# lgleznah/mort

Measured on AMD Instinct MI355X. Metric: Msamples/sec (width x height x spp/s), Scene 1 1200x675, higher is better.
Workload: dtype f32; 1 GPU; Scene 1 (random-spheres cover) 1200x675, 500 spp nominal = 484 effective, depth 20, megakernel, seed 69420, host LCG scene; mode=mega, partition=rows/8 interleaved over 1 rank(s)

## Files before the change

mort_amd/csrc/hip/debug.hip:

```cpp
#include <hip/hip_runtime.h>

#include <array>
#include <cstring>
#include <thread>
#include <vector>

#include "mort_hip.h"
#include "mega_bvh.h"
#include "scene_blob.h"
#include "mort_ctx.h"
#include "world_images.h"
#include "dev_radiance.h"
#include "query_common.h"

#pragma clang fp contract(off)

extern "C" int mort_hip_debug_wave_log(mort_ctx *c, unsigned long long *out, size_t max_waves) {
    if (!c || !out || !c->d_wave_log) return 0;
    hipSetDevice(c->device);
    quiesce(c);
    const size_t n = c->wave_log_waves < max_waves ? c->wave_log_waves : max_waves;
    if (hipMemcpy(out, c->d_wave_log, n * 16 * sizeof(unsigned long long), hipMemcpyDeviceToHost) != hipSuccess) return 0;
    return (int)n;
}
// ... 255 lines not shown
    if (hipSetDevice(device) != hipSuccess) return MORT_ERR_NO_DEVICE;
    float *d_in = nullptr;
    unsigned long long *d_out = nullptr;
    int st = MORT_OK;
    if (hipMalloc((void **)&d_in, n * per * sizeof(float)) != hipSuccess || hipMalloc((void **)&d_out, 16 * sizeof(unsigned long long)) != hipSuccess) st = MORT_ERR_NOMEM;
    if (st == MORT_OK && (hipMemcpy(d_in, in, n * per * sizeof(float), hipMemcpyHostToDevice) != hipSuccess ||
                          hipMemset(d_out, 0, 16 * sizeof(unsigned long long)) != hipSuccess)) st = MORT_ERR_HIP;
    if (st == MORT_OK) {
        const size_t blocks = (n + 255) / 256;
        exact_forms_kernel<<<dim3((unsigned)(blocks < 4096 ? blocks : 4096)), dim3(256)>>>(what, d_in, n, d_out);
        if (hipGetLastError() != hipSuccess || hipDeviceSynchronize() != hipSuccess ||
            hipMemcpy(out, d_out, 16 * sizeof(unsigned long long), hipMemcpyDeviceToHost) != hipSuccess) st = MORT_ERR_HIP;
    }
    if (d_in) (void)hipFree(d_in);
    if (d_out) (void)hipFree(d_out);
    if (caller_device >= 0 && caller_device != device) (void)hipSetDevice(caller_device);
    return st;
}

extern "C" int mort_hip_debug_bvh_lds_levels(const mort_world *w, int *out) {
    if (!w || !out) return MORT_ERR_INVALID;
    SceneBlob sb;
    const int st = build_scene_blob(w, sb);
    if (st != MORT_OK) return st;
    const mortc::Compiled &o = sb.comp;
    for (int i = 0; i < 4; i++) out[i] = 0;
    if (!one_sphere_bvh(o) || o.own_nodes.empty() || o.own_nodes4.empty()) return MORT_OK;
    BvhImages im;
    build_bvh_images(o, im);
    if (!im.fits) return MORT_OK;
    const uint32_t levels = (uint32_t)(o.own4_stack > 1 ? o.own4_stack : 1) + MORT_BVH_TSTACK_SPARE;
    const int shapes[3] = {1024, 768, 256};
    out[0] = (int)im.fb.size();
    for (int k = 0; k < 3; k++) { uint32_t a = 0, b = 0; out[1 + k] = state_lds_levels((uint32_t)im.fb.size(), shapes[k], levels, 1024u, a, b); }
    return MORT_OK;
}


__device__ __forceinline__ int mort_f2i_select(float x) {
    const bool in_range = (x > -2147483648.0f) && (x < 2147483648.0f);
    const int t = (int)(in_range ? x : 0.0f);
    return (x != x) ? 0 : (x >= 2147483648.0f) ? 2147483647 : (x <= -2147483648.0f) ? (-2147483647 - 1) : t;
}
static __global__ void __launch_bounds__(256) f2i_all_kernel(unsigned long long *out) {
    const uint32_t first = blockIdx.x * 256u + threadIdx.x;
    uint32_t differ = 0, lowest = 0xffffffffu;
    for (uint32_t k = 0; k < 4096u; k++) {
        const uint32_t bits = first + (k << 20);
        const float x = __uint_as_float(bits);
        if (mort_f2i(x) != mort_f2i_select(x)) { differ++; lowest = bits < lowest ? bits : lowest; }
    }
    atomicAdd(&out[2], 4096ull);
    if (differ) { atomicAdd(&out[0], (unsigned long long)differ); atomicMin(&out[1], (unsigned long long)lowest); }
}
static __global__ void __launch_bounds__(256) f2i_list_kernel(const uint32_t *bits, size_t n, int *res) {
    const size_t i = (size_t)blockIdx.x * 256 + threadIdx.x;
    if (i < n) res[i] = mort_f2i(__uint_as_float(bits[i]));
}

extern "C" int mort_hip_debug_f2i_device(int device, const uint32_t *bits, size_t n, int *res, unsigned long long *out) {
    if (!out || (n && (!bits || !res)) || n > ((size_t)1 << 28)) return MORT_ERR_INVALID;
    int caller_device = -1;
    if (hipGetDevice(&caller_device) != hipSuccess) caller_device = -1;
    if (hipSetDevice(device) != hipSuccess) return MORT_ERR_NO_DEVICE;
    uint32_t *d_bits = nullptr;
    int *d_res = nullptr;
    unsigned long long *d_out = nullptr;
// ... 514 lines not shown
```

mort_amd/csrc/hip/mega_bvh.h:

```cpp
#ifndef MORT_MEGA_BVH_H
#define MORT_MEGA_BVH_H

#include "dev_render.h"


struct FastArgs {
    RenderArgs r;
    const unsigned char *hot_src;
    uint32_t hot_bytes;
    uint32_t off_nodes4, off_leafrecs, off_lambert, off_metal, off_diel, off_dlight, off_iso, off_solid, off_checker;
    uint32_t off_tstack;
    int node_first, node_count;
    unsigned int *next_q;
    int tiles_x, tiles_total;
    uint32_t off_stack;
    int stack_lds_depth;
    const unsigned *tile_order;
    int gen_tiles;
    int spread_shift;
    unsigned *tile_cost;
    int th_s, th_l, t_keep;
    int sub;
    float *vaccum;
    float4 *deep;
// ... 370 lines not shown
#define TS_AT(ptr) (*(ptr))
    const DLambert *lambert = (const DLambert *)(lds + BU_U(L.off_lambert));
    const DMetal *metal = (const DMetal *)(lds + BU_U(L.off_metal));
    const DDielectric *dielectric = (const DDielectric *)(lds + BU_U(L.off_diel));
    const DLambert *dlight = (const DLambert *)(lds + BU_U(L.off_dlight));
    const DLambert *isotropic = (const DLambert *)(lds + BU_U(L.off_iso));
    const DSolid *solid = (const DSolid *)(lds + BU_U(L.off_solid));
    const DChecker *checker = (const DChecker *)(lds + BU_U(L.off_checker));

    const int node_first = BU_I(L.node_first), node_end = node_first + BU_I(L.node_count);
    const int th_s = BU_I(L.th_s), th_l = BU_I(L.th_l), t_keep = BU_I(L.t_keep);
    const int sqrt_spp = BU_I(L.r.sqrt_spp), bounce_limit = BU_I(L.r.bounce_limit);
    const float bg_x = BU_F(L.r.background.x), bg_y = BU_F(L.r.background.y), bg_z = BU_F(L.r.background.z);
    const int spp = sqrt_spp * sqrt_spp;
    const unsigned total_q = (unsigned)BU_I(L.tiles_total) * 64u;

    int state = ((int)(threadIdx.x & 63u) < BU_I(L.lane_cap)) ? ST_S : ST_DONE, kind = K_NEWPIX;
    int xy = 0, lofs = 0;
    Rng rng; rng.d = rng.v0 = rng.v1 = rng.v2 = rng.v3 = rng.v4 = 0; rng.draws = 0;
    V3 pixel_color = mk(0, 0, 0);
    int s_ij = 0, iter = 0;
    uint32_t segments = 0;
    Ray ray; ray.o = mk(0, 0, 0); ray.d = mk(0, 0, 1); ray.tm = 0;
    float ray_time0 = 0;
    OwnRay orr; orr.ix = orr.iy = orr.iz = 1; orr.mx = orr.my = orr.mz = 0; orr.band = 0; orr.invlen = 1;
    float ray_a = 1, closest = 0;
    float ray_a_rcp = 1;
    int best = -1;
    uint32_t node = 0;
    unsigned short *spa = ts_base;
    int flags = 0;
    DeepPtr stack_deep = (DeepPtr)BU_P(L.deep) + ((size_t)blockIdx.x * BLOCK + threadIdx.x);
    const size_t deep_stride = (size_t)gridDim.x * BLOCK;
    unsigned long long ident_mask = 0ull;
    float4 *stack_lds = (float4 *)(lds + BU_U(L.off_stack));
    const int DL = BU_I(L.stack_lds_depth);
#ifdef MORT_PROFILE_STATES
    unsigned long long *const counters_p = fap->r.counters;
    unsigned long long prof[6] = {0, 0, 0, 0, 0, 0};
    unsigned long long prof_truns = 0;
    unsigned long long profc[8] = {0, 0, 0, 0, 0, 0, 0, 0};
    unsigned long long ps0 = 0, ps1;
#define PROFS0() do { ps0 = __builtin_readcyclecounter(); } while (0)
#define PROFS(i) do { ps1 = __builtin_readcyclecounter(); profc[i] += ps1 - ps0; ps0 = ps1; } while (0)
    unsigned long long pt0 = __builtin_readcyclecounter(), pt1;
    const unsigned long long prof_r0 = __builtin_amdgcn_s_memrealtime();
#define PROF(i, lanes) do { prof[2 * (i)] += 1; prof[2 * (i) + 1] += (unsigned long long)(lanes); } while (0)
    unsigned long long profb[12] = {0, 0, 0, 0, 0, 0, 0, 0, 0, 0, 0, 0};
#ifdef MORT_PROFILE_FINE
#define PROFB(i) do { } while (0)
    unsigned long long proff[12] = {0, 0, 0, 0, 0, 0, 0, 0, 0, 0, 0, 0};
#define PROFF(i) do { ps1 = __builtin_readcyclecounter(); proff[i] += ps1 - ps0; profc[4] += ps1 - ps0; ps0 = ps1; } while (0)
#else
#define PROFF(i) do { } while (0)
#define PROFB(i) do { const unsigned long long m_ = __ballot(1); if ((int)(threadIdx.x & 63) == __ffsll((long long)m_) - 1) { \
        atomicAdd(&counters_p[18 + 2 * (i)], 1ull); atomicAdd(&counters_p[19 + 2 * (i)], (unsigned long long)__popcll(m_)); } } while (0)
#endif
#define PROFC(i) do { pt1 = __builtin_readcyclecounter(); profc[i] += pt1 - pt0; pt0 = pt1; } while (0)
#else
#define PROF(i, lanes) do { } while (0)
#define PROFB(i) do { } while (0)
#define PROFF(i) do { } while (0)
#define PROFC(i) do { } while (0)
#define PROFS0() do { } while (0)
#define PROFS(i) do { } while (0)
#endif

    int leader = -1;
    const bool drain_rounds = DRAIN && BU_I(L.drain_rounds) == 1;
    const bool live_thresholds = BU_I(L.drain_rounds) == 3;
    bool running = true;
    while (running) {
      int nS = 0;
      for (;;) {
        const unsigned long long mT = __ballot(state == ST_T);
        const unsigned long long mL = __ballot(state == ST_L);
        const unsigned long long mS = __ballot(state == ST_S);
        if ((mT | mL | mS) == 0ull) { running = false; break; }
        const int nT = __popcll(mT), nL = __popcll(mL);
        nS = __popcll(mS);
        int pick;
// ... 130 lines not shown
                        atomicAdd(&fap->r.counters[3], 1ull);
                        const RefHit h = reference_walk(fap->r.sc.nodes, node_first, node_end, fap->r.sc.spheres, ray.o.x, ray.o.y, ray.o.z,
                                                        ray.d.x, ray.d.y, ray.d.z, ray.tm, ray_a);
                        best = h.best; closest = h.closest;
                    }
                    PROFF(0);
                REGION("S:hitrecord");
                    if (best < 0) {
                        final_value = mk(bg_x, bg_y, bg_z);
                        kind = K_FINISH;
                    } else {
                        DSphere sp;
                        if (need_ref) sp = fap->r.sc.spheres[best];
                        else {
                            const float4 *lp = leafrecs + (best >> 16) + ((best & 0x8000) ? 2 : 0);
                            const float4 s0 = lp[0], s1 = lp[1];
                            sp.cx = s0.x; sp.cy = s0.y; sp.cz = s0.z; sp.radius = s0.w; sp.vx = s1.x; sp.vy = s1.y; sp.vz = s1.z; sp.mat = __float_as_uint(s1.w);
                        }
                        const V3 p = ray_at(ray, closest);
                        const V3 outward = vdiv(vsub(p, sphere_center(sp, ray.tm)), sp.radius);
                        const bool front_face = vdot(ray.d, outward) < 0;
                        const V3 normal = front_face ? outward : vneg(outward);
                        const int mtype = DREF_TYPE(sp.mat), midx = DREF_IDX(sp.mat);
                        PROFF(1);
                        StackEntry e;
                        if (mtype == MORT_MAT_METAL) {
                REGION("S:metal");
                            PROFB(0);
                            const DMetal m = metal[midx];
                            V3 reflected = reflect(ray.d, normal);
                            reflected = vadd(vunit(reflected), vscale(m.fuzz, random_unit_vector(rng)));
                            ray.o = p; ray.d = reflected;
                            e.kx = 1.0f * m.r; e.ky = 1.0f * m.g; e.kz = 1.0f * m.b; e.rp = 1.0f;
                            PROFF(2);
                        } else if (mtype == MORT_MAT_DIELECTRIC) {
                REGION("S:dielectric");
                            PROFB(1);
                            const DDielectric m = dielectric[midx];
                            const float refraction_ratio = front_face ? m.inv_ior : m.ior;
                            const V3 unit_direction = vunit(ray.d);
                            const float cos_theta = (float)mort_fmin((double)vdot(vneg(unit_direction), normal), 1.0);
                            const float sin_theta = (float)mort_sqrt(1.0 - (double)(cos_theta * cos_theta));
                            const bool cant_refract = (double)(refraction_ratio * sin_theta) > 1.0;
                            V3 direction;
                            if (cant_refract || reflectance(cos_theta, refraction_ratio) > random_float(rng))
                                direction = reflect(unit_direction, normal);
                            else
                                direction = refract(unit_direction, normal, refraction_ratio);
                            ray.o = p; ray.d = direction;
                            e.kx = 1.0f; e.ky = 1.0f; e.kz = 1.0f; e.rp = 1.0f;
                            ident_mask |= (1ull << iter);
                            PROFF(3);
                        } else if (mtype == MORT_MAT_LAMBERTIAN || mtype == MORT_MAT_ISOTROPIC) {
                REGION("S:lambertian");
                            PROFB(2);
                            const bool lamb = (mtype == MORT_MAT_LAMBERTIAN);
                            const DLambert m = lamb ? lambert[midx] : isotropic[midx];
                            V3 attenuation = mk(m.r, m.g, m.b);
                            if (m.tex != 0) {
                                uint32_t tex = m.tex;
                                bool resolved = false;
                                for (int guard = 0; guard < 8 && !resolved; guard++) {
                                    const int tt = DREF_TYPE(tex), ti = DREF_IDX(tex);
                                    if (tt == MORT_TEXTURE_SOLID) { const DSolid sc = solid[ti]; attenuation = mk(sc.r, sc.g, sc.b); resolved = true; }
                                    else if (tt == MORT_TEXTURE_CHECKER) {
                                        const DChecker c = checker[ti];
                                        const int xi = mort_f2i(mort_floorf(c.inv_scale * p.x));
                                        const int yi = mort_f2i(mort_floorf(c.inv_scale * p.y));
                                        const int zi = mort_f2i(mort_floorf(c.inv_scale * p.z));
                                        tex = ((xi + yi + zi) % 2 == 0) ? c.even : c.odd;
                                    } else break;
                                }
                                if (!resolved) {
                                    const V3Ret c = texture_value_uv(&fap->r.sc, tex, outward.x, outward.y, outward.z, p.x, p.y, p.z);
                                    attenuation = mk(c.x, c.y, c.z);
                                }
                            }
                            PROFF(4);
                REGION("S:lamb_scatter");
                            V3 dir;
                            float mat_pdf, scattering_pdf;
                            if (lamb) {
                                const Onb uvw = onb_from_w(normal);
                                dir = onb_local(uvw, random_cosine_direction(rng));
                                const V3 ud = vunit(dir);
                                const float cosine_theta = vdot(ud, uvw.w);
                                mat_pdf = mort_fmaxf(0, (float)((double)cosine_theta / 3.1415926));
                                const float cos_theta = vdot(normal, ud);
                                scattering_pdf = (cos_theta < 0) ? 0.0f : (float)((double)cos_theta / 3.141592565);
                            } else {
                                dir = random_unit_vector(rng);
                                mat_pdf = (float)(1 / (4 * 3.1415926));
                                scattering_pdf = (float)(1 / (4 * 3.1415926));
                            }
                            ray.o = p; ray.d = dir; ray.tm = ray_time0;
                            e.kx = scattering_pdf * attenuation.x; e.ky = scattering_pdf * attenuation.y; e.kz = scattering_pdf * attenuation.z;
                            e.rp = 1 / mat_pdf;
                            PROFF(5);
                        } else {
                REGION("S:light");
                            V3 emission = mk(0, 0, 0);
                            if (mtype == MORT_MAT_DIFFUSE_LIGHT && front_face) {
                                const DLambert m = dlight[midx];
                                if (m.tex == 0) emission = mk(m.r, m.g, m.b);
                                else { const V3Ret c = texture_value_uv(&fap->r.sc, m.tex, outward.x, outward.y, outward.z, p.x, p.y, p.z); emission = mk(c.x, c.y, c.z); }
                            }
                            final_value = emission;
                            kind = K_FINISH;
                            PROFF(6);
                        }
                REGION("S:stackstore");
                        if (kind == K_SHADE) {
                            if (!((ident_mask >> iter) & 1ull)) {
                                float4 e4; e4.x = e.kx; e4.y = e.ky; e4.z = e.kz; e4.w = e.rp;
                                if (iter < DL) stack_lds[iter * BLOCK + threadIdx.x] = e4;
                                else stack_deep[(size_t)(iter - DL) * deep_stride] = DeepEntry{e4.x, e4.y, e4.z, e4.w};
                            }
                            iter++;
                            if (iter >= bounce_limit) { final_value = mk(0, 0, 0); kind = K_FINISH; }
                        }
                    }
                }
                REGION("S:finish");
                PROFS(4);
                if (kind == K_FINISH) {
                    PROFB(3);
                    if (iter > 0) {
                        unsigned long long todo = ~ident_mask & (iter >= 64 ? ~0ull : ((1ull << iter) - 1ull));
                        if ((ident_mask >> (iter - 1)) & 1ull) final_value = vadd(mk(0, 0, 0), final_value);
                        while (todo != 0ull) {
                            const int lvl = 63 - __builtin_clzll(todo);
                            todo &= ~(1ull << lvl);
                            StackEntry e;
                            if (lvl < DL) { const float4 e4 = stack_lds[lvl * BLOCK + threadIdx.x]; e.kx = e4.x; e.ky = e4.y; e.kz = e4.z; e.rp = e4.w; }
                            else { const DeepEntry e4 = stack_deep[(size_t)(lvl - DL) * deep_stride]; e.kx = e4.x; e.ky = e4.y; e.kz = e4.z; e.rp = e4.w; }
                            const V3 t = vmul(mk(e.kx, e.ky, e.kz), final_value);
                            final_value = vadd(mk(0, 0, 0), vscale(e.rp, t));
                        }
                        iter = 0;
                    }
                    ident_mask = 0ull;
                    pixel_color = vadd(pixel_color, final_value);
                    s_ij++;
                    bool more;
                    if constexpr (SUB) {
                        more = (s_ij & 0xffff) != sqrt_spp;
                    } else {
                        if ((s_ij & 0xffff) == sqrt_spp) s_ij = (s_ij & ~0xffff) + 0x10000;
                        more = (s_ij >> 16) < sqrt_spp;
                    }
                    if (more) {
                        kind = K_NEWSAMPLE;
                    } else {
                        pixel_write<PROBE, SUB>(fap, pixel_color.x, pixel_color.y, pixel_color.z, lofs, segments, rng.draws, rng.d, rng.v0, rng.v1, rng.v2, rng.v3, rng.v4);
                        kind = K_NEWPIX;
                    }
                }
                REGION("S:newpix");
                PROFS(5);
                if (kind == K_NEWPIX) {
                    const PixelFetch pf = pixel_fetch<SUB>(fap, total_q);
                    if (!pf.got) state = ST_DONE;
                    else {
                        xy = pf.xy; lofs = pf.lofs;
                        rng.d = pf.d; rng.v0 = pf.v0; rng.v1 = pf.v1; rng.v2 = pf.v2; rng.v3 = pf.v3; rng.v4 = pf.v4;
                        rng.draws = 0;
                        pixel_color = mk(0, 0, 0);
                        s_ij = SUB ? ((pf.got - 1) << 16) : 0; segments = 0;
                        kind = (spp > 0) ? K_NEWSAMPLE : K_FINISH;
                        if (spp <= 0) {
                            final_value = mk(0, 0, 0);
                        }
                    }
                }
// ... 3 lines not shown
                    if (kind == K_NEWSAMPLE) {
                        PROFB(4);
                        ray = get_ray(s_cam, xy & 0xffff, (xy >> 16) & 0x7fff, rng, s_ij & 0xffff, s_ij >> 16);
                        ray_time0 = ray.tm;
                        iter = 0;
                        kind = K_SHADE;
                        if (bounce_limit <= 0) { final_value = mk(0, 0, 0); kind = K_FINISH; }
                    }
                REGION("S:setup");
                    if (kind == K_SHADE) {
                        ray_a = vlen2(ray.d);
                        ray_a_rcp = div_prepare(ray_a).r;
                        orr.ix = 1.0f / ray.d.x; orr.iy = 1.0f / ray.d.y; orr.iz = 1.0f / ray.d.z;
                        orr.mx = ray.o.x * orr.ix; orr.my = ray.o.y * orr.iy; orr.mz = ray.o.z * orr.iz;
                        const float mm = __builtin_fmaxf(__builtin_fmaxf(mort_fabsf(orr.mx), mort_fabsf(orr.my)), mort_fabsf(orr.mz));
                        orr.band = mm * 4.76837158203125e-07f;
                        orr.invlen = 1.01f / mort_sqrtf(ray_a);
                        const bool ordinary = own_inv_ok(orr.ix) && own_inv_ok(orr.iy) && own_inv_ok(orr.iz) && (mm < 1e30f);
                        closest = __builtin_inff();
                        best = -1;
                        node = 0; spa = ts_base;
                        flags = ordinary ? FL_SIGNS(own_sign_offset(orr.ix), own_sign_offset(orr.iy), own_sign_offset(orr.iz)) : FL_REF;
                        segments++;
                        state = ordinary ? ST_T : ST_S;
                    }
                }
            }
                REGION("S:end");
            if (DRAIN && __ballot(state == ST_DONE) != 0ull) {
                unsigned key = (state <= ST_S) ? ((unsigned)((s_ij >> 16) * sqrt_spp + (s_ij & 0xffff)) << 6) | (threadIdx.x & 63u) : 0xffffffffu;
                for (int off = 32; off > 0; off >>= 1) { const unsigned o = (unsigned)__shfl_xor((int)key, off); key = o < key ? o : key; }
                leader = (key == 0xffffffffu) ? -1 : __builtin_amdgcn_readfirstlane((int)(key & 63u));
            }
            PROFS(7);
            PROFC(2);
        }
    }
    if ((threadIdx.x & 63) == 0) {
#ifdef MORT_PROFILE_STATES
#ifdef MORT_PROFILE_FINE
        for (int k = 0; k < 12; k++) atomicAdd(&counters_p[18 + k], proff[k]);
#endif
        for (int k = 0; k < 6; k++) atomicAdd(&counters_p[4 + k], prof[k]);
        atomicAdd(&counters_p[30], prof_truns);
        for (int k = 0; k < 4; k++) atomicAdd(&counters_p[10 + k], profc[k]);
        for (int k = 4; k < 8; k++) atomicAdd(&counters_p[14 + k - 4], profc[k]);
        if (fap->wave_log) {
            unsigned long long *w = fap->wave_log + 16 * ((size_t)blockIdx.x * (BLOCK / 64) + (threadIdx.x >> 6));
            w[0] = blockIdx.x; w[1] = threadIdx.x >> 6; w[2] = __builtin_amdgcn_s_memrealtime() - prof_r0;
            w[3] = prof[0]; w[4] = prof[2]; w[5] = 0; w[6] = prof[4]; w[7] = profc[0]; w[8] = profc[1]; w[9] = 0; w[10] = profc[2]; w[11] = profc[3];
        }
        (void)profb;
#endif
    }
}

#endif
```

mort_amd/csrc/hip/mort_hip.hip:

```cpp
#include <hip/hip_runtime.h>

#include <climits>
#include <cmath>
#include <cstdio>
#include <cstdlib>
#include <cstring>

#include "mort_hip.h"
#include "dev_pixel.h"
#include "scene_blob.h"
#include "mort_internal.h"
#include "mort_ctx.h"
#include "world_images.h"
#include "mega_gen.h"
#include "wave_gen.h"

#pragma clang fp contract(off)


#ifndef MORT_GENERIC_WAVES
#define MORT_GENERIC_WAVES 4
#endif
#ifndef MORT_MEGA_LDS_LEVELS
#define MORT_MEGA_LDS_LEVELS 9
// ... 104 lines not shown
        HIPCHK(c, hipMemsetAsync(c->d_counters, 0, 96 * sizeof(unsigned long long), s));
        c->cost_key = key;
    }
    HIPCHK(c, mort_tile_sort_desc(c->d_tile_cost, c->d_tile_keys, c->d_tile_iota, c->d_tile_order, c->d_sort_tmp, c->sort_tmp_bytes, tiles, s));
    fa.prio_dev = nullptr;
    if (fa.heavy_mod > 0) {
        HIPCHK(c, mort_tile_heavy_count(c->d_tile_keys, tiles, (unsigned)c->heavy_percent, (unsigned)(tiles / 2 > 0 ? tiles / 2 : 1),
                                        (const unsigned long long *)(c->d_prio_count + 4), (unsigned long long)grid * (unsigned long long)FB, c->d_prio_count, s));
        fa.prio_dev = c->d_prio_count;
    }
    HIPCHK(c, hipMemsetAsync(c->d_tile_cost, 0, (size_t)tiles * sizeof(unsigned), s));
    fa.tile_order = c->d_tile_order; fa.tile_cost = c->d_tile_cost;
    fa.tile_key_sum = key_sum;
    fa.gen_tiles = grid * (FB / 64);
    fa.spread_shift = chain_bound ? 0 : 6;
    knob_int(std::getenv("MORT_SPREAD_SHIFT"), fa.spread_shift);
    if (fa.spread_shift >= 6 || fa.spread_shift < 0) fa.gen_tiles = 0;
    if (timed) HIPCHK(c, hipEventRecord(c->ev0, s));
    return MORT_OK;
}


static void fast_args_base(const mort_ctx *c, const mort_camera *cam, const RenderArgs &a, FastArgs &fa, const void *image, uint32_t image_bytes,
                           int tiles, bool sub) {
    fa.r = a;
    fa.hot_src = (const unsigned char *)image; fa.hot_bytes = image_bytes;
    fa.next_q = (unsigned int *)(c->d_counters + 2);
    fa.tiles_x = (a.width + 7) / 8; fa.tiles_total = tiles;
    if (sub) { fa.sub = cam->sqrt_spp; fa.vaccum = c->d_vaccum; fa.r.states = c->d_substates; }
    fa.lane_cap = 64;
    knob_int_in(std::getenv("MORT_LANE_CAP"), 1, 64, fa.lane_cap);
}

static int state_setup(mort_ctx *c, const mort_camera *cam, FastArgs &fa, const void *kern, int FB, uint32_t tstack_levels, int dl_cap,
                       int per_cu_cap, const char *too_big, hipStream_t s, size_t &lds_bytes, int &grid) {
    uint32_t static_lds = 1024;
    { hipFuncAttributes fattr; if (hipFuncGetAttributes(&fattr, kern) == hipSuccess) static_lds = (uint32_t)((fattr.sharedSizeBytes + 1023) & ~(size_t)1023); }
    uint32_t tstack_off = 0, stack_off = 0;
    int dl = state_lds_levels(fa.hot_bytes, FB, tstack_levels, static_lds, tstack_off, stack_off);
    fa.off_tstack = tstack_off;
    if (dl < 0) { c->last_error = too_big; return MORT_ERR_CAPACITY; }
    if (dl > dl_cap) dl = dl_cap;
    fa.off_stack = stack_off; fa.stack_lds_depth = dl;
    lds_bytes = (size_t)stack_off + (size_t)dl * FB * 16;
    HIPCHK(c, hipFuncSetAttribute(kern, hipFuncAttributeMaxDynamicSharedMemorySize, (int)lds_bytes));
    int per_cu = 0;
    if (hipOccupancyMaxActiveBlocksPerMultiprocessor(&per_cu, kern, FB, lds_bytes) != hipSuccess || per_cu < 1) per_cu = 1;
    if (per_cu > per_cu_cap) per_cu = per_cu_cap;
    grid = c->num_cus * per_cu;
    const int want_blocks = (int)(((long long)fa.tiles_total * 64 + FB - 1) / FB);
    if (grid > want_blocks) grid = want_blocks;
    if (grid < 1) grid = 1;
    const int deep_levels = cam->bounce_limit > dl ? cam->bounce_limit - dl : 0;
    const int st = ensure_buf(c, &c->d_deep, &c->deep_cap, (size_t)(deep_levels > 0 ? deep_levels : 1) * (size_t)grid * (size_t)FB * sizeof(float4));
    if (st != MORT_OK) return st;
    fa.deep = (float4 *)c->d_deep;
    fa.wave_log = nullptr;
    if (std::getenv("MORT_WAVE_LINES")) {
        c->wave_log_waves = (size_t)grid * (size_t)(FB / 64);
        if (ensure_buf(c, &c->d_wave_log, &c->wave_log_cap, c->wave_log_waves * 16 * sizeof(unsigned long long)) == MORT_OK) {
            hipMemsetAsync(c->d_wave_log, 0, c->wave_log_waves * 16 * sizeof(unsigned long long), s);
            fa.wave_log = (unsigned long long *)c->d_wave_log;
        }
    }
    return MORT_OK;
}

typedef void (*bvh_kernel_t)(const FastArgs);
static bvh_kernel_t bvh_kernel(int FB, bool probe, bool drain, bool sub) {
    if (!sub) switch (FB) {
        case 1024: return !probe ? mega_bvh_kernel<1024, false, false> : mega_bvh_kernel<1024, true, false>;
        case 768: return probe ? mega_bvh_kernel<768, true, false> : drain ? mega_bvh_kernel<768, false, true> : mega_bvh_kernel<768, false, false>;
// ... 7 lines not shown

static int launch_bvh(mort_ctx *c, const mort_camera *cam, const RenderArgs &a, int tiles, bool sub, bool timed, hipStream_t s, LaunchPlan &plan) {
    FastArgs fa;
    std::memset(&fa, 0, sizeof fa);
    fast_args_base(c, cam, a, fa, c->d_fast, c->fast_bytes, tiles, sub);
    const BvhOffsets &o = c->bvh;
    fa.off_nodes4 = o.f_nodes4; fa.off_leafrecs = o.f_leafrecs; fa.off_lambert = o.f_lambert; fa.off_metal = o.f_metal;
    fa.off_diel = o.f_diel; fa.off_dlight = o.f_dlight; fa.off_iso = o.f_iso; fa.off_solid = o.f_solid; fa.off_checker = o.f_checker;
    fa.node_first = 0; fa.node_count = c->sc.n_nodes;
    const long long lanes_wanted = (long long)tiles * 64;
    const double px_per_lane = (double)lanes_wanted / ((double)c->num_cus * 768.0);
    int FB = MORT_FAST_BLOCK;
    if (!knob_int(std::getenv("MORT_FAST_BLOCK_SIZE"), FB)) {
        const int cand[4] = {768, 512, 384, 256};
        FB = 256;
        const bool wide_ok = lanes_wanted >= 2ll * 1024 * c->num_cus;
        for (int k = (px_per_lane < 1.5 && !sub) ? 1 : 0; k < 4; k++) if (lanes_wanted >= (long long)cand[k] * c->num_cus) { FB = cand[k]; break; }
        if (wide_ok) FB = 1024;
    }
    if (FB == 1024 && !bvh_wide_block_fits(fa.hot_bytes, c->own4_stack)) FB = 768;
    if (FB != 1024 && FB != 768 && FB != 512 && FB != 384) FB = 256;
    fa.drain_rounds = 3;
    { int dm = 0; if (knob_int(std::getenv("MORT_BVH_DRAIN"), dm)) fa.drain_rounds = dm == 2 ? 1 : dm == 3 ? 3 : 0; }
    bool chain_bound = px_per_lane < 1.5 && !sub;
    if (!sub) knob_flag(std::getenv("MORT_CHAIN_BOUND"), chain_bound);
    if (FB == 1024) chain_bound = false;
    const bvh_kernel_t kern = bvh_kernel(FB, false, chain_bound, sub), kern_probe = bvh_kernel(FB, true, false, false);
    fa.th_s = MORT_TH_S; fa.th_l = MORT_TH_L; fa.t_keep = MORT_T_KEEP;
    { int th[3]; if (knob_ints(std::getenv("MORT_THRESHOLDS"), 3, 1, th)) { fa.th_s = th[0]; fa.th_l = th[1]; fa.t_keep = th[2]; } }
    int per_cu_cap = INT_MAX;
    knob_int_in(std::getenv("MORT_FAST_BLOCKS_PER_CU"), 1, INT_MAX, per_cu_cap);
    size_t lds_bytes = 0;
    int grid = 0;
    int st = state_setup(c, cam, fa, (const void *)kern, FB, (uint32_t)c->own4_stack + MORT_BVH_TSTACK_SPARE, 12, per_cu_cap, "BVH image does not fit one CU's LDS", s, lds_bytes, grid);
    if (st != MORT_OK) return st;
    st = prepare_tile_order(c, cam, a, fa, tiles, grid, FB, chain_bound, sub, timed, s, [&](const FastArgs &pa) {
        hipError_t e_ = hipFuncSetAttribute((const void *)kern_probe, hipFuncAttributeMaxDynamicSharedMemorySize, (int)lds_bytes);
        if (e_ != hipSuccess) return e_;
        hipLaunchKernelGGL(kern_probe, dim3(grid), dim3(FB), lds_bytes, s, pa);
        return hipGetLastError();
    });
    if (st != MORT_OK) return st;
    hipLaunchKernelGGL(kern, dim3(grid), dim3(FB), lds_bytes, s, fa);
    HIPCHK(c, hipGetLastError());
    plan.kernel = (const void *)kern; plan.block = FB; plan.lds_bytes = (int)lds_bytes;
    std::snprintf(plan.name, sizeof plan.name, "mega_bvh_kernel<%d, false, %s, %s>", FB, chain_bound ? "true" : "false", sub ? "true" : "false");
    return MORT_OK;
}

static int launch_gen(mort_ctx *c, const mort_camera *cam, const RenderArgs &a, int tiles, bool sub, bool timed, hipStream_t s, LaunchPlan &plan) {
    GenArgs ga = c->gen;
    FastArgs &fa = ga.f;
    fast_args_base(c, cam, a, fa, c->d_gen, c->gen_bytes, tiles, sub);
    const long long lanes_wanted = (long long)tiles * 64;
    int FB = 768;
    bool heavy_default = false;
    if (sub || !knob_int(std::getenv("MORT_GEN_BLOCK_SIZE"), FB)) {
        const double ppl = (double)lanes_wanted / ((double)c->num_cus * 768.0);
        FB = ppl >= 8.0 ? 1024 : (lanes_wanted >= 512ll * c->num_cus) ? 512 : 256;
        if (ppl < 8.0 && lanes_wanted >= 32ll * 1024 && !std::getenv("MORT_GEN_NO_HEAVY")) { FB = 1024; heavy_default = true; }
    }
    if (FB != 1024 && FB != 768 && FB != 512 && FB != 256) FB = 256;
    if (FB == 1024 && (size_t)c->gen_bytes + 16u + (size_t)MORT_OWN_STACK * 1024u * 2u + 2048u > 160u * 1024u) FB = 768;
    if (sub && FB > 512) FB = 512;
    fa.th_s = 28; fa.th_l = 20; fa.t_keep = 4; ga.th_m = 56;
    fa.heavy_mod = 0; fa.heavy_num = 0; fa.heavy_cap = 64; c->heavy_percent = 50;
    if (heavy_default && FB == 1024 && !sub) { fa.heavy_mod = 3; fa.heavy_num = 2; fa.heavy_cap = 12; }
    { int hv[4];
      if (!sub && knob_ints(std::getenv("MORT_GEN_HEAVY"), 4, 1, hv) && hv[1] <= hv[0] && hv[2] <= 64 && hv[3] <= 100) {
          fa.heavy_mod = hv[0]; fa.heavy_num = hv[1]; fa.heavy_cap = hv[2]; c->heavy_percent = hv[3]; } }
    ga.drain_mode = 3;
    knob_int_in(std::getenv("MORT_GEN_DRAIN"), 0, 3, ga.drain_mode);
    { int th[4]; if (knob_ints(std::getenv("MORT_GEN_THRESHOLDS"), 4, 1, th)) { fa.th_s = th[0]; fa.th_l = th[1]; fa.t_keep = th[2]; ga.th_m = th[3]; } }
    const gen_kernel_t kern = mort_gen_kernel(FB, ga.prims_in_lds != 0, sub);
    int dl_cap = 12;
    if (knob_int(std::getenv("MORT_GEN_DL"), dl_cap) && dl_cap < 0) dl_cap = 0;
    size_t lds_bytes = 0;
    int grid = 0;
    int st = state_setup(c, cam, fa, (const void *)kern, FB, MORT_OWN_STACK, dl_cap, INT_MAX, "unified-tree image does not fit one CU's LDS", s, lds_bytes, grid);
    if (st != MORT_OK) return st;
    st = prepare_tile_order(c, cam, a, fa, tiles, grid, FB, false, sub, timed, s, [&](const FastArgs &pa) {
        GenArgs pg = ga;
        pg.f = pa;
        pg.probe = 1;
        hipError_t e_ = hipFuncSetAttribute((const void *)kern, hipFuncAttributeMaxDynamicSharedMemorySize, (int)lds_bytes);
        if (e_ != hipSuccess) return e_;
        hipLaunchKernelGGL(kern, dim3(grid), dim3(FB), lds_bytes, s, pg);
        return hipGetLastError();
    });
    if (st != MORT_OK) return st;
    if (fa.tile_order) {
        int k_prio = 0;
        knob_int(std::getenv("MORT_GEN_PRIO_LANES"), k_prio);
        if (k_prio > 0 && ga.drain_mode == 1) {
            const long long waves = (long long)grid * (FB / 64);
            long long pt = (waves * k_prio + 63) / 64;
            if (pt > tiles / 4) pt = tiles / 4;
            fa.prio_tiles = (int)pt; fa.prio_lanes = k_prio;
        }
    }
    hipLaunchKernelGGL(kern, dim3(grid), dim3(FB), lds_bytes, s, ga);
    HIPCHK(c, hipGetLastError());
    if (fa.heavy_mod > 0 && c->d_prio_count && std::getenv("MORT_GEN_HEAVY_DEBUG")) {
        unsigned h[4] = {0, 0, 0, 0};
        HIPCHK(c, hipStreamSynchronize(s));
        HIPCHK(c, hipMemcpy(h, c->d_prio_count, 16, hipMemcpyDeviceToHost));
        std::fprintf(stderr, "[heavy] head tiles %u of %d, lanes %d\n", h[0], tiles, grid * FB);
    }
    if (fa.heavy_mod > 0 && c->d_prio_count)
        HIPCHK(c, hipMemcpyAsync(c->d_prio_count + 4, c->d_counters, 96 * sizeof(unsigned long long), hipMemcpyDeviceToDevice, s));
    plan.kernel = (const void *)kern; plan.block = FB; plan.lds_bytes = (int)lds_bytes;
    std::snprintf(plan.name, sizeof plan.name, "mega_gen_kernel<%d, %s, %s>", FB, ga.prims_in_lds ? "true" : "false", sub ? "true" : "false");
// ... 42 lines not shown
                         cnt[4 + k] ? (double)cnt[12 + k] / (double)cnt[4 + k] : 0.0);
        std::fprintf(stderr, "[wf_trav sched] cycles %5.1f%%   fronts %d\n", 100.0 * (double)cnt[15] / tot, c->wf_fronts);
        std::fprintf(stderr, "[wf_trav waves] %llu waves, mean lifetime %.1f us, in-loop cycles per wave %.0f\n", cnt[21],
                     cnt[21] ? (double)cnt[20] / (double)cnt[21] * 0.01 : 0.0, cnt[21] ? tot / (double)cnt[21] : 0.0);
    } else if (fam == FAM_GEN) {
        const char *nm[4] = {"T", "L", "M", "S"};
        unsigned long long segs = cnt[0];
        for (int k = 0; k < 32; k++) segs += cnt[32 + 2 * k];
        const double tot = (double)(cnt[12] + cnt[13] + cnt[14] + cnt[15] + cnt[16]);
        for (int k = 0; k < 4; k++)
            std::fprintf(stderr, "[gen %s] %12llu wave-steps  lanes %5.1f%%  cycles %5.1f%% (%.0f/step)\n", nm[k], cnt[4 + 2 * k],
                         cnt[4 + 2 * k] ? 100.0 * (double)cnt[5 + 2 * k] / (64.0 * (double)cnt[4 + 2 * k]) : 0.0, 100.0 * (double)cnt[12 + k] / tot,
                         cnt[4 + 2 * k] ? (double)cnt[12 + k] / (double)cnt[4 + 2 * k] : 0.0);
        std::fprintf(stderr, "[gen S parts, cycles per S step] scan+decode %.0f  shade call %.0f  stack store %.0f  finish %.0f  newpix %.0f  newray %.0f\n", (double)cnt[24] / (double)cnt[10],
                     (double)cnt[25] / (double)cnt[10], (double)cnt[20] / (double)cnt[10], (double)cnt[21] / (double)cnt[10], (double)cnt[22] / (double)cnt[10], (double)cnt[23] / (double)cnt[10]);
        std::fprintf(stderr, "[gen sched] cycles %5.1f%%; leaf loop: %.2f iterations per L step, %.1f lanes per iteration; scans %llu; steps per segment: T %.2f L %.2f M %.2f S %.2f\n",
                     100.0 * (double)cnt[16] / tot, cnt[6] ? (double)cnt[17] / (double)cnt[6] : 0.0, cnt[17] ? (double)cnt[18] / (double)cnt[17] : 0.0, cnt[3],
                     (double)cnt[5] / (double)(segs + 1), (double)cnt[7] / (double)(segs + 1), (double)cnt[9] / (double)(segs + 1), (double)cnt[11] / (double)(segs + 1));
    } else if (fam == FAM_BVH) {
        const char *nm[3] = {"T", "L", "S"};
        for (int k = 0; k < 3; k++)
            std::fprintf(stderr, "[states] %s: %llu wave-steps, %llu lane-steps, utilisation %.1f%%\n", nm[k], cnt[4 + 2 * k], cnt[5 + 2 * k],
                         cnt[4 + 2 * k] ? 100.0 * (double)cnt[5 + 2 * k] / (64.0 * (double)cnt[4 + 2 * k]) : 0.0);
        std::fprintf(stderr, "[states] box-step runs: %llu (%.1f steps per run)\n", cnt[30], cnt[30] ? (double)cnt[4] / (double)cnt[30] : 0.0);
        const double tot = (double)(cnt[10] + cnt[11] + cnt[12] + cnt[13]);
        std::fprintf(stderr, "[cycles] T %.1f%% (%.0f/step)  L %.1f%% (%.0f/step)  S %.1f%% (%.0f/step)  sched %.1f%%  total wave-cycles %.3g\n",
                     100.0 * cnt[10] / tot, (double)cnt[10] / (double)cnt[4], 100.0 * cnt[11] / tot, (double)cnt[11] / (double)cnt[6],
                     100.0 * cnt[12] / tot, (double)cnt[12] / (double)cnt[8], 100.0 * cnt[13] / tot, tot);
#ifdef MORT_PROFILE_FINE
        std::fprintf(stderr, "[S shade parts, cycles/step] verify %.0f  hit record %.0f  metal %.0f  dielectric %.0f  lambert texture %.0f  lambert scatter %.0f  light %.0f  (rest of 'shade' below: stack store)\n",
                     (double)cnt[18] / (double)cnt[8], (double)cnt[19] / (double)cnt[8], (double)cnt[20] / (double)cnt[8], (double)cnt[21] / (double)cnt[8],
                     (double)cnt[22] / (double)cnt[8], (double)cnt[23] / (double)cnt[8], (double)cnt[24] / (double)cnt[8]);
#else
        const char *bn[6] = {"metal", "dielectric", "lambertian", "finish", "get_ray", "unwind iteration"};
        for (int k = 0; k < 6; k++)
            std::fprintf(stderr, "[S branch] %-16s entered in %5.1f%% of S steps (x%.2f), %4.1f lanes when entered\n", bn[k],
                         100.0 * (double)cnt[18 + 2 * k] / (double)cnt[8], (double)cnt[18 + 2 * k] / (double)cnt[8],
                         cnt[18 + 2 * k] ? (double)cnt[19 + 2 * k] / (double)cnt[18 + 2 * k] : 0.0);
#endif
        std::fprintf(stderr, "[S parts, cycles/step] shade %.0f  finish %.0f  newpix %.0f  newsample+setup %.0f\n", (double)cnt[14] / (double)cnt[8],
                     (double)cnt[15] / (double)cnt[8], (double)cnt[16] / (double)cnt[8], (double)cnt[17] / (double)cnt[8]);
    }
}
#endif

static int collect_stats(mort_ctx *c, const LaunchPlan &plan, int W, int local_rows, int sqrt_spp, bool has_accum, mort_stats *stats) {
    HIPCHK(c, hipEventSynchronize(c->ev1));
    float ms = 0;
    HIPCHK(c, hipEventElapsedTime(&ms, c->ev0, c->ev1));
    unsigned long long cnt[96] = {0};
    HIPCHK(c, hipMemcpy(cnt, c->d_counters, sizeof cnt, hipMemcpyDeviceToHost));
#ifdef MORT_PROFILE_STATES
    print_profile(c, plan.fam, cnt);
#endif
    const bool wave = plan.fam == FAM_WAVE || plan.fam == FAM_WAVE_GEN;
    std::memset(stats, 0, sizeof *stats);
    stats->seconds = ms * 1e-3;
    for (int k = 0; k < 32; k++) { cnt[0] += cnt[32 + 2 * k]; cnt[1] += cnt[33 + 2 * k]; }
    stats->segments = cnt[0];
    stats->rng_draws = cnt[1];
    stats->reference_walks = (plan.fam == FAM_BVH || plan.fam == FAM_GEN) ? cnt[3] : 0;
    stats->pixels = (uint64_t)W * (uint64_t)local_rows;
    stats->eff_samples = stats->pixels * (uint64_t)(sqrt_spp * sqrt_spp);
    stats->algorithmic_hbm_bytes = stats->pixels * (uint64_t)(100 + (has_accum ? 12 : 0));
    stats->scene_in_lds = plan.fam != FAM_MEGA ? 1 : 0;
    if (wave) stats->algorithmic_hbm_bytes += 240ull * stats->segments;
    stats->local_rows = local_rows;
    std::snprintf(stats->kernel_name, sizeof stats->kernel_name, "%s", plan.name);
    hipFuncAttributes fattr;
    if (hipFuncGetAttributes(&fattr, plan.kernel) == hipSuccess) {
        stats->kernel_vgprs = fattr.numRegs;
// ... 102 lines not shown
```

mort_amd/csrc/hip/world_images.h:

```cpp
#ifndef MORT_WORLD_IMAGES_H
#define MORT_WORLD_IMAGES_H

#include <cstring>
#include <vector>

#include "scene_blob.h"
#include "mega_gen.h"

static inline bool one_sphere_bvh(const mortc::Compiled &o) { return o.items.size() == 1 && o.items[0].kind == ITEM_BVH && o.quads.empty(); }

#define MORT_BVH_IMAGE_MAX (72 * 1024)
struct BvhOffsets {
    uint32_t f_nodes4, f_leafrecs, f_lambert, f_metal, f_diel, f_dlight, f_iso, f_solid, f_checker, t_nodes2, t_leaves, t_spheres;
};
struct BvhImages {
    std::vector<unsigned char> fb, tb;
    BvhOffsets off;
    bool fits;
};
static inline void build_bvh_images(const mortc::Compiled &o, BvhImages &im) {
    std::vector<unsigned char> &fb = im.fb, &tb = im.tb;
    BvhOffsets &f = im.off;
    f.f_nodes4 = (uint32_t)place(fb, o.own_nodes4); f.f_leafrecs = (uint32_t)place(fb, o.own_leafrecs);
    f.f_lambert = (uint32_t)place(fb, o.lambert); f.f_metal = (uint32_t)place(fb, o.metal); f.f_diel = (uint32_t)place(fb, o.dielectric);
// ... 19 lines not shown
    size_t table_bytes, prim_bytes, lds_part, o_ranks;
    bool fits;
};
static inline void build_gen_image(const mortc::Compiled &o, GenImage &gi) {
    std::vector<unsigned char> &gb = gi.gb;
    GenArgs &g = gi.g;
    std::memset(&g, 0, sizeof g);
    g.o_nodes = (uint32_t)place(gb, o.g_nodes); g.o_leaves = g.o_nodes; g.o_entries = (uint32_t)place(gb, o.g_entries);
    g.o_chains = (uint32_t)place(gb, o.g_chains); g.o_xforms = (uint32_t)place(gb, o.xforms);
    g.o_items = (uint32_t)place(gb, o.items); g.o_subitems = (uint32_t)place(gb, o.subitems); g.o_media = (uint32_t)place(gb, o.media);
    g.o_lambert = (uint32_t)place(gb, o.lambert); g.o_metal = (uint32_t)place(gb, o.metal); g.o_diel = (uint32_t)place(gb, o.dielectric);
    g.o_dlight = (uint32_t)place(gb, o.dlight); g.o_iso = (uint32_t)place(gb, o.isotropic);
    g.o_solid = (uint32_t)place(gb, o.solid); g.o_checker = (uint32_t)place(gb, o.checker); g.o_image = (uint32_t)place(gb, o.image);
    g.o_lfirst = (uint32_t)place(gb, std::vector<int>(o.list_first, o.list_first + MORT_NUM_HITTABLE_LIST));
    g.o_lcount = (uint32_t)place(gb, std::vector<int>(o.list_count, o.list_count + MORT_NUM_HITTABLE_LIST));
    gi.table_bytes = gb.size();
    gi.prim_bytes = o.spheres.size() * sizeof(DSphere) + o.quads.size() * sizeof(DQuad) + o.wspheres.size() * sizeof(DSphere) +
                    o.wquads.size() * sizeof(DQuad) + (o.list_types.size() + o.list_idxs.size()) * sizeof(int) + 6 * 32;
    if (gi.table_bytes + gi.prim_bytes <= MORT_GEN_PRIMS_LDS_MAX) {
        g.prims_in_lds = 1;
        g.o_spheres = (uint32_t)place(gb, o.spheres); g.o_quads = (uint32_t)place(gb, o.quads);
        g.o_wspheres = (uint32_t)place(gb, o.wspheres); g.o_wquads = (uint32_t)place(gb, o.wquads);
        g.o_ltypes = (uint32_t)place(gb, o.list_types); g.o_lidxs = (uint32_t)place(gb, o.list_idxs);
    }
    gb.resize((gb.size() + 15) & ~(size_t)15, 0);
    gi.lds_part = gb.size();
    gi.o_ranks = place(gb, o.g_ranks);
    g.n_spheres = (int)o.spheres.size();
    g.root = o.g_root; g.first_medium = o.g_first_medium; g.n_chains = (int)(o.g_chains.size() / 2);
    g.gx = o.g_c[0]; g.gy = o.g_c[1]; g.gz = o.g_c[2]; g.gR = o.g_R; g.mnear = o.g_mnear; g.kmin = o.g_kmin;
    gi.fits = gi.lds_part <= MORT_GEN_IMAGE_MAX;
}

static inline int state_lds_levels(uint32_t hot_bytes, int FB, uint32_t tstack_levels, uint32_t static_lds, uint32_t &tstack_off, uint32_t &stack_off) {
    tstack_off = (hot_bytes + 15u) & ~15u;
    stack_off = tstack_off + tstack_levels * (uint32_t)FB * 2u;
    int groups_per_cu = FB >= 768 ? 1 : 768 / FB;
    while (groups_per_cu > 1 && (long long)(stack_off + static_lds) * groups_per_cu > 160ll * 1024) groups_per_cu--;
    const long long room = (160ll * 1024 - (long long)static_lds * groups_per_cu) / groups_per_cu - (long long)stack_off;
    if (room < 0) return -1;
    const int dl = (int)(room / ((long long)FB * 16));
    return dl > 12 ? 12 : dl;
}

#endif
```

Baseline: 4465 Msamples/s.

## Replace indexed bounce stack with LDS ring buffer spilling oldest entries to HBM

Measured after the change: 4521 Msamples/s, median of 6. +1.3%, better.

```diff
diff --git a/mort_amd/csrc/hip/debug.hip b/mort_amd/csrc/hip/debug.hip
--- a/mort_amd/csrc/hip/debug.hip
+++ b/mort_amd/csrc/hip/debug.hip
@@ -311,7 +311,7 @@
     const uint32_t levels = (uint32_t)(o.own4_stack > 1 ? o.own4_stack : 1) + MORT_BVH_TSTACK_SPARE;
     const int shapes[3] = {1024, 768, 256};
     out[0] = (int)im.fb.size();
-    for (int k = 0; k < 3; k++) { uint32_t a = 0, b = 0; out[1 + k] = state_lds_levels((uint32_t)im.fb.size(), shapes[k], levels, 1024u, a, b); }
+    for (int k = 0; k < 3; k++) { uint32_t a = 0, b = 0; out[1 + k] = state_lds_levels((uint32_t)im.fb.size(), shapes[k], levels, 1024u, 1, a, b); }
     return MORT_OK;
 }
 
diff --git a/mort_amd/csrc/hip/mega_bvh.h b/mort_amd/csrc/hip/mega_bvh.h
--- a/mort_amd/csrc/hip/mega_bvh.h
+++ b/mort_amd/csrc/hip/mega_bvh.h
@@ -426,9 +426,14 @@
     int flags = 0;
     DeepPtr stack_deep = (DeepPtr)BU_P(L.deep) + ((size_t)blockIdx.x * BLOCK + threadIdx.x);
     const size_t deep_stride = (size_t)gridDim.x * BLOCK;
-    unsigned long long ident_mask = 0ull;
-    float4 *stack_lds = (float4 *)(lds + BU_U(L.off_stack));
+    int nst = 0;
     const int DL = BU_I(L.stack_lds_depth);
+    float4 *const stack_lds = (float4 *)(lds + BU_U(L.off_stack));
+#define RING_AT(k) stack_lds[(k) * BLOCK + threadIdx.x]
+#ifndef MORT_BVH_UNWIND_P
+#define MORT_BVH_UNWIND_P 2
+#endif
+    static_assert(MORT_BVH_UNWIND_P == 0 || MORT_BVH_UNWIND_P == 2 || MORT_BVH_UNWIND_P == 3, "MORT_BVH_UNWIND_P");
 #ifdef MORT_PROFILE_STATES
     unsigned long long *const counters_p = fap->r.counters;
     unsigned long long prof[6] = {0, 0, 0, 0, 0, 0};
@@ -441,6 +446,8 @@
     const unsigned long long prof_r0 = __builtin_amdgcn_s_memrealtime();
 #define PROF(i, lanes) do { prof[2 * (i)] += 1; prof[2 * (i) + 1] += (unsigned long long)(lanes); } while (0)
     unsigned long long profb[12] = {0, 0, 0, 0, 0, 0, 0, 0, 0, 0, 0, 0};
+    int uw_l = 0, uw_h = 0;
+    unsigned long long prof_uw[3] = {0, 0, 0};
 #ifdef MORT_PROFILE_FINE
 #define PROFB(i) do { } while (0)
     unsigned long long proff[12] = {0, 0, 0, 0, 0, 0, 0, 0, 0, 0, 0, 0};
@@ -637,6 +644,7 @@
                             reflected = vadd(vunit(reflected), vscale(m.fuzz, random_unit_vector(rng)));
                             ray.o = p; ray.d = reflected;
                             e.kx = 1.0f * m.r; e.ky = 1.0f * m.g; e.kz = 1.0f * m.b; e.rp = 1.0f;
+                            nst &= ~1;
                             PROFF(2);
                         } else if (mtype == MORT_MAT_DIELECTRIC) {
                 REGION("S:dielectric");
@@ -654,7 +662,7 @@
                                 direction = refract(unit_direction, normal, refraction_ratio);
                             ray.o = p; ray.d = direction;
                             e.kx = 1.0f; e.ky = 1.0f; e.kz = 1.0f; e.rp = 1.0f;
-                            ident_mask |= (1ull << iter);
+                            nst |= 1;
                             PROFF(3);
                         } else if (mtype == MORT_MAT_LAMBERTIAN || mtype == MORT_MAT_ISOTROPIC) {
                 REGION("S:lambertian");
@@ -701,6 +709,7 @@
                             ray.o = p; ray.d = dir; ray.tm = ray_time0;
                             e.kx = scattering_pdf * attenuation.x; e.ky = scattering_pdf * attenuation.y; e.kz = scattering_pdf * attenuation.z;
                             e.rp = 1 / mat_pdf;
+                            nst &= ~1;
                             PROFF(5);
                         } else {
                 REGION("S:light");
@@ -716,10 +725,17 @@
                         }
                 REGION("S:stackstore");
                         if (kind == K_SHADE) {
-                            if (!((ident_mask >> iter) & 1ull)) {
+                            if (!(nst & 1)) {
                                 float4 e4; e4.x = e.kx; e4.y = e.ky; e4.z = e.kz; e4.w = e.rp;
-                                if (iter < DL) stack_lds[iter * BLOCK + threadIdx.x] = e4;
-                                else stack_deep[(size_t)(iter - DL) * deep_stride] = DeepEntry{e4.x, e4.y, e4.z, e4.w};
+                                const int n = nst >> 8;
+                                int ring = (nst >> 1) & 15;
+                                if (n >= DL) {
+                                    const float4 old = RING_AT(ring);
+                                    stack_deep[(size_t)(n - DL) * deep_stride] = DeepEntry{old.x, old.y, old.z, old.w};
+                                }
+                                RING_AT(ring) = e4;
+                                ring = ring + 1 == DL ? 0 : ring + 1;
+                                nst = ((n + 1) << 8) | (ring << 1);
                             }
                             iter++;
                             if (iter >= bounce_limit) { final_value = mk(0, 0, 0); kind = K_FINISH; }
@@ -730,21 +746,60 @@
                 PROFS(4);
                 if (kind == K_FINISH) {
                     PROFB(3);
-                    if (iter > 0) {
-                        unsigned long long todo = ~ident_mask & (iter >= 64 ? ~0ull : ((1ull << iter) - 1ull));
-                        if ((ident_mask >> (iter - 1)) & 1ull) final_value = vadd(mk(0, 0, 0), final_value);
-                        while (todo != 0ull) {
-                            const int lvl = 63 - __builtin_clzll(todo);
-                            todo &= ~(1ull << lvl);
-                            StackEntry e;
-                            if (lvl < DL) { const float4 e4 = stack_lds[lvl * BLOCK + threadIdx.x]; e.kx = e4.x; e.ky = e4.y; e.kz = e4.z; e.rp = e4.w; }
-                            else { const DeepEntry e4 = stack_deep[(size_t)(lvl - DL) * deep_stride]; e.kx = e4.x; e.ky = e4.y; e.kz = e4.z; e.rp = e4.w; }
-                            const V3 t = vmul(mk(e.kx, e.ky, e.kz), final_value);
-                            final_value = vadd(mk(0, 0, 0), vscale(e.rp, t));
+                    if (nst != 0) {
+#define UNWIND_LEVEL(v) do { const V3 t_ = vmul(mk((v).x, (v).y, (v).z), final_value); final_value = vadd(mk(0, 0, 0), vscale((v).w, t_)); } while (0)
+#define UNWIND_LEVEL_IF(c, v) do { const V3 t_ = vmul(mk((v).x, (v).y, (v).z), final_value); const V3 f_ = vadd(mk(0, 0, 0), vscale((v).w, t_)); \
+        final_value.x = (c) ? f_.x : final_value.x; final_value.y = (c) ? f_.y : final_value.y; final_value.z = (c) ? f_.z : final_value.z; } while (0)
+                        if (nst & 1) final_value = vadd(mk(0, 0, 0), final_value);
+                        const int n = nst >> 8;
+                        int ring = (nst >> 1) & 15;
+                        int nd = n > DL ? n - DL : 0;
+                        int nr = n - nd;
+                        int di = nd;
+#ifdef MORT_PROFILE_STATES
+                        uw_l = nr; uw_h = nd;
+#endif
+#if MORT_BVH_UNWIND_P > 0
+                        DeepEntry q0 = DeepEntry{0, 0, 0, 0}, q1 = q0;
+                        if (nd > 0) { di--; q0 = stack_deep[(size_t)di * deep_stride]; }
+                        if (nd > 1) { di--; q1 = stack_deep[(size_t)di * deep_stride]; }
+#if MORT_BVH_UNWIND_P > 2
+                        DeepEntry q2 = q0;
+                        if (nd > 2) { di--; q2 = stack_deep[(size_t)di * deep_stride]; }
+#endif
+#endif
+                        while (nr > 0) {
+                            const int r1 = (ring == 0 ? DL : ring) - 1;
+                            const int r2 = (r1 == 0 ? DL : r1) - 1;
+                            const float4 a = RING_AT(r1), b = RING_AT(r2);
+                            ring = nr > 1 ? r2 : r1;
+                            UNWIND_LEVEL(a);
+                            UNWIND_LEVEL_IF(nr > 1, b);
+                            nr -= 2;
                         }
+#if MORT_BVH_UNWIND_P == 0
+                        while (nd > 0) { nd--; const DeepEntry v = stack_deep[(size_t)nd * deep_stride]; UNWIND_LEVEL(v); }
+                        (void)di;
+#else
+                        while (nd > 0) {
+                            UNWIND_LEVEL(q0);
+                            if (nd > MORT_BVH_UNWIND_P) { di--; q0 = stack_deep[(size_t)di * deep_stride]; }
+                            nd--;
+                            UNWIND_LEVEL_IF(nd > 0, q1);
+                            if (nd > MORT_BVH_UNWIND_P) { di--; q1 = stack_deep[(size_t)di * deep_stride]; }
+                            nd--;
+#if MORT_BVH_UNWIND_P > 2
+                            UNWIND_LEVEL_IF(nd > 0, q2);
+                            if (nd > MORT_BVH_UNWIND_P) { di--; q2 = stack_deep[(size_t)di * deep_stride]; }
+                            nd--;
+#endif
+                        }
+#endif
+#undef UNWIND_LEVEL
+#undef UNWIND_LEVEL_IF
                         iter = 0;
+                        nst = 0;
                     }
-                    ident_mask = 0ull;
                     pixel_color = vadd(pixel_color, final_value);
                     s_ij++;
                     bool more;
@@ -814,6 +869,15 @@
                 for (int off = 32; off > 0; off >>= 1) { const unsigned o = (unsigned)__shfl_xor((int)key, off); key = o < key ? o : key; }
                 leader = (key == 0xffffffffu) ? -1 : __builtin_amdgcn_readfirstlane((int)(key & 63u));
             }
+#ifdef MORT_PROFILE_STATES
+            {
+                int sl = uw_l, sh = uw_h, mx = uw_l + uw_h;
+                for (int off = 32; off > 0; off >>= 1) { sl += __shfl_xor(sl, off); sh += __shfl_xor(sh, off); const int o = __shfl_xor(mx, off); mx = o > mx ? o : mx; }
+                prof_uw[0] += (unsigned long long)__builtin_amdgcn_readfirstlane(sl); prof_uw[1] += (unsigned long long)__builtin_amdgcn_readfirstlane(sh);
+                prof_uw[2] += (unsigned long long)__builtin_amdgcn_readfirstlane(mx);
+                uw_l = 0; uw_h = 0;
+            }
+#endif
             PROFS(7);
             PROFC(2);
         }
@@ -825,12 +889,14 @@
 #endif
         for (int k = 0; k < 6; k++) atomicAdd(&counters_p[4 + k], prof[k]);
         atomicAdd(&counters_p[30], prof_truns);
+        atomicAdd(&counters_p[28], prof_uw[0]); atomicAdd(&counters_p[29], prof_uw[1]); atomicAdd(&counters_p[31], prof_uw[2]);
         for (int k = 0; k < 4; k++) atomicAdd(&counters_p[10 + k], profc[k]);
         for (int k = 4; k < 8; k++) atomicAdd(&counters_p[14 + k - 4], profc[k]);
         if (fap->wave_log) {
             unsigned long long *w = fap->wave_log + 16 * ((size_t)blockIdx.x * (BLOCK / 64) + (threadIdx.x >> 6));
             w[0] = blockIdx.x; w[1] = threadIdx.x >> 6; w[2] = __builtin_amdgcn_s_memrealtime() - prof_r0;
             w[3] = prof[0]; w[4] = prof[2]; w[5] = 0; w[6] = prof[4]; w[7] = profc[0]; w[8] = profc[1]; w[9] = 0; w[10] = profc[2]; w[11] = profc[3];
+            w[12] = prof_uw[0]; w[13] = prof_uw[1]; w[14] = prof_uw[2]; w[15] = profc[5];
         }
         (void)profb;
 #endif
diff --git a/mort_amd/csrc/hip/mort_hip.hip b/mort_amd/csrc/hip/mort_hip.hip
--- a/mort_amd/csrc/hip/mort_hip.hip
+++ b/mort_amd/csrc/hip/mort_hip.hip
@@ -160,12 +160,12 @@
     knob_int_in(std::getenv("MORT_LANE_CAP"), 1, 64, fa.lane_cap);
 }
 
-static int state_setup(mort_ctx *c, const mort_camera *cam, FastArgs &fa, const void *kern, int FB, uint32_t tstack_levels, int dl_cap,
+static int state_setup(mort_ctx *c, const mort_camera *cam, FastArgs &fa, const void *kern, int FB, uint32_t tstack_levels, int dl_min, int dl_cap,
                        int per_cu_cap, const char *too_big, hipStream_t s, size_t &lds_bytes, int &grid) {
     uint32_t static_lds = 1024;
     { hipFuncAttributes fattr; if (hipFuncGetAttributes(&fattr, kern) == hipSuccess) static_lds = (uint32_t)((fattr.sharedSizeBytes + 1023) & ~(size_t)1023); }
     uint32_t tstack_off = 0, stack_off = 0;
-    int dl = state_lds_levels(fa.hot_bytes, FB, tstack_levels, static_lds, tstack_off, stack_off);
+    int dl = state_lds_levels(fa.hot_bytes, FB, tstack_levels, static_lds, dl_min, tstack_off, stack_off);
     fa.off_tstack = tstack_off;
     if (dl < 0) { c->last_error = too_big; return MORT_ERR_CAPACITY; }
     if (dl > dl_cap) dl = dl_cap;
@@ -239,7 +239,7 @@
     knob_int_in(std::getenv("MORT_FAST_BLOCKS_PER_CU"), 1, INT_MAX, per_cu_cap);
     size_t lds_bytes = 0;
     int grid = 0;
-    int st = state_setup(c, cam, fa, (const void *)kern, FB, (uint32_t)c->own4_stack + MORT_BVH_TSTACK_SPARE, 12, per_cu_cap, "BVH image does not fit one CU's LDS", s, lds_bytes, grid);
+    int st = state_setup(c, cam, fa, (const void *)kern, FB, (uint32_t)c->own4_stack + MORT_BVH_TSTACK_SPARE, 1, 12, per_cu_cap, "BVH image does not fit one CU's LDS", s, lds_bytes, grid);
     if (st != MORT_OK) return st;
     st = prepare_tile_order(c, cam, a, fa, tiles, grid, FB, chain_bound, sub, timed, s, [&](const FastArgs &pa) {
         hipError_t e_ = hipFuncSetAttribute((const void *)kern_probe, hipFuncAttributeMaxDynamicSharedMemorySize, (int)lds_bytes);
@@ -284,7 +284,7 @@
     if (knob_int(std::getenv("MORT_GEN_DL"), dl_cap) && dl_cap < 0) dl_cap = 0;
     size_t lds_bytes = 0;
     int grid = 0;
-    int st = state_setup(c, cam, fa, (const void *)kern, FB, MORT_OWN_STACK, dl_cap, INT_MAX, "unified-tree image does not fit one CU's LDS", s, lds_bytes, grid);
+    int st = state_setup(c, cam, fa, (const void *)kern, FB, MORT_OWN_STACK, 0, dl_cap, INT_MAX, "unified-tree image does not fit one CU's LDS", s, lds_bytes, grid);
     if (st != MORT_OK) return st;
     st = prepare_tile_order(c, cam, a, fa, tiles, grid, FB, false, sub, timed, s, [&](const FastArgs &pa) {
         GenArgs pg = ga;
@@ -393,11 +393,14 @@
                      (double)cnt[18] / (double)cnt[8], (double)cnt[19] / (double)cnt[8], (double)cnt[20] / (double)cnt[8], (double)cnt[21] / (double)cnt[8],
                      (double)cnt[22] / (double)cnt[8], (double)cnt[23] / (double)cnt[8], (double)cnt[24] / (double)cnt[8]);
 #else
-        const char *bn[6] = {"metal", "dielectric", "lambertian", "finish", "get_ray", "unwind iteration"};
-        for (int k = 0; k < 6; k++)
+        const char *bn[5] = {"metal", "dielectric", "lambertian", "finish", "get_ray"};
+        for (int k = 0; k < 5; k++)
             std::fprintf(stderr, "[S branch] %-16s entered in %5.1f%% of S steps (x%.2f), %4.1f lanes when entered\n", bn[k],
                          100.0 * (double)cnt[18 + 2 * k] / (double)cnt[8], (double)cnt[18 + 2 * k] / (double)cnt[8],
                          cnt[18 + 2 * k] ? (double)cnt[19 + 2 * k] / (double)cnt[18 + 2 * k] : 0.0);
+        std::fprintf(stderr, "[S branch] unwind iteration: %.2f levels from LDS + %.2f from HBM per S step (%.1f %% from HBM), the step's deepest lane unwinds %.2f\n",
+                     (double)cnt[28] / (double)cnt[8], (double)cnt[29] / (double)cnt[8], cnt[28] + cnt[29] ? 100.0 * (double)cnt[29] / (double)(cnt[28] + cnt[29]) : 0.0,
+                     (double)cnt[31] / (double)cnt[8]);
 #endif
         std::fprintf(stderr, "[S parts, cycles/step] shade %.0f  finish %.0f  newpix %.0f  newsample+setup %.0f\n", (double)cnt[14] / (double)cnt[8],
                      (double)cnt[15] / (double)cnt[8], (double)cnt[16] / (double)cnt[8], (double)cnt[17] / (double)cnt[8]);
diff --git a/mort_amd/csrc/hip/world_images.h b/mort_amd/csrc/hip/world_images.h
--- a/mort_amd/csrc/hip/world_images.h
+++ b/mort_amd/csrc/hip/world_images.h
@@ -75,14 +75,15 @@
     gi.fits = gi.lds_part <= MORT_GEN_IMAGE_MAX;
 }
 
-static inline int state_lds_levels(uint32_t hot_bytes, int FB, uint32_t tstack_levels, uint32_t static_lds, uint32_t &tstack_off, uint32_t &stack_off) {
+static inline int state_lds_levels(uint32_t hot_bytes, int FB, uint32_t tstack_levels, uint32_t static_lds, int min_levels, uint32_t &tstack_off, uint32_t &stack_off) {
     tstack_off = (hot_bytes + 15u) & ~15u;
     stack_off = tstack_off + tstack_levels * (uint32_t)FB * 2u;
     int groups_per_cu = FB >= 768 ? 1 : 768 / FB;
-    while (groups_per_cu > 1 && (long long)(stack_off + static_lds) * groups_per_cu > 160ll * 1024) groups_per_cu--;
+    while (groups_per_cu > 1 && (long long)(stack_off + static_lds + (uint32_t)min_levels * (uint32_t)FB * 16u) * groups_per_cu > 160ll * 1024) groups_per_cu--;
     const long long room = (160ll * 1024 - (long long)static_lds * groups_per_cu) / groups_per_cu - (long long)stack_off;
     if (room < 0) return -1;
     const int dl = (int)(room / ((long long)FB * 16));
+    if (dl < min_levels) return -1;
     return dl > 12 ? 12 : dl;
 }
 
```
